# xkuubix/MonteCarlo-Gated-MIL

Measured on AMD Instinct MI355X. Metric: bags/sec × MCDO-samples (T=100) at N=2048,d=512; 1/2/4/8-GPU + %HBM roofline, higher is better.
Workload: dtype bf16

## Files before the change

montecarlo-gated-mil_amd/csrc/mcgmil_kernels.h:

```cpp
#pragma once
#include "mcgmil_device.h"

namespace mcgmil {

struct GateParams {
    const void* H;
    long long ldh;
    const int32_t* bag_off;
    int B, T, L, D, C, G, P;
    long long total_samples;
    const void* Wp;
    uint32_t wp_bytes;
    const float* bv;
    const float* bu;
    const float* wa;
    const float* ba;
    float sf, sa;
    uint32_t thr_f, thr_a;
    uint32_t thrx_f;
    uint32_t k0, k1;
    uint32_t bag_base;
    int t_base;
    const uint32_t* bag_ids;
    const int32_t* tile_bag;
    int uniform_rows;
    const uint8_t* keep_feat;
    const uint8_t* keep_att;
    float* logits;
    float* zz;
    float* Y;
    float* A;
    const int32_t* region_off;
    int region_t;
    unsigned long long* stamps;
    unsigned long long* clock;
    long long tile_row0;
};

constexpr int kClockSlots = 1024;
__device__ __forceinline__ void clock_probe(const GateParams& p, int i) {
    if (p.clock && threadIdx.x == 0 && blockIdx.x < (unsigned)kClockSlots) {
        const unsigned long long t = __builtin_amdgcn_s_memtime();
        const unsigned long long r = __builtin_amdgcn_s_memrealtime();
        p.clock[(size_t)blockIdx.x * 4 + 2 * i] = t;
        p.clock[(size_t)blockIdx.x * 4 + 2 * i + 1] = r;
    }
}

#ifdef MCGMIL_STAMPS
#define MCGMIL_STAMP(p, i)                                                                 \
    do {                                                                                    \
        __builtin_amdgcn_sched_barrier(0);                                                  \
        if (threadIdx.x == 0 && (p).stamps)                                                 \
            (p).stamps[(size_t)blockIdx.x * 8 + (i)] = __builtin_amdgcn_s_memtime();        \
        __builtin_amdgcn_sched_barrier(0);                                                  \
    } while (0)
#else
#define MCGMIL_STAMP(p, i) do {} while (0)
#endif


constexpr int kGateThreads = 512;
constexpr int kGateWaves = kGateThreads / kWave;
constexpr int kRowInfo = 6;


template <int BM, int RV = BM>
__device__ __forceinline__ void fill_row_table(const GateParams& p, long long R0, int* rinfo) {
    const int tid = threadIdx.x;
    if (tid >= BM) return;
    const long long R = tid < RV ? R0 + tid : p.total_samples;
    int hrow = -1, t = 0, n = 0, bag = 0, Nb = 0;
    const bool narrow = p.total_samples <= 0xFFFFFFFFll;
    if (R < p.total_samples && p.uniform_rows > 0) {
        const long long per_bag = (long long)p.T * p.uniform_rows;
        Nb = p.uniform_rows;
        if (narrow) {
            const uint32_t r = (uint32_t)R, pb = (uint32_t)per_bag;
            bag = (int)(r / pb);
            const uint32_t local = r - (uint32_t)bag * pb;
            t = (int)(local / (uint32_t)Nb);
            n = (int)(local - (uint32_t)t * (uint32_t)Nb);
        } else {
            bag = (int)(R / per_bag);
            const long long local = R - (long long)bag * per_bag;
            t = (int)(local / Nb);
            n = (int)(local - (long long)t * Nb);
        }
        hrow = bag * Nb + n;
    } else if (R < p.total_samples) {
        if (p.tile_bag) {
            bag = p.tile_bag[R0 / BM];
            while ((long long)p.T * p.bag_off[bag + 1] <= R) ++bag;
        } else {
            bag = find_bag(p.bag_off, p.B, p.T, R);
        }
        const int ob = p.bag_off[bag];
        Nb = p.bag_off[bag + 1] - ob;
        const long long local = R - (long long)p.T * ob;
        if (narrow) {
            t = (int)((uint32_t)local / (uint32_t)Nb);
            n = (int)((uint32_t)local - (uint32_t)t * (uint32_t)Nb);
        } else {
            t = (int)(local / Nb);
            n = (int)(local - (long long)t * Nb);
        }
        hrow = ob + n;
    }
    int* ri = rinfo + kRowInfo * tid;
    ri[0] = hrow; ri[1] = t; ri[2] = n; ri[3] = bag; ri[4] = Nb;
    ri[5] = (int)(p.bag_ids ? p.bag_ids[bag] : p.bag_base + (uint32_t)bag);
}

#ifndef MCGMIL_KERNELS_TEMPLATES_ONLY
__global__ void plan_tiles_kernel(const int32_t* bag_off, int B, int T, long long total_samples,
                                  int BM, long long tiles, int32_t* tile_bag) {
    const long long i = (long long)blockIdx.x * blockDim.x + threadIdx.x;
    if (i >= tiles) return;
    const long long R = i * BM;
    tile_bag[i] = R < total_samples ? find_bag(bag_off, B, T, R) : 0;
}
#endif

__device__ __forceinline__ float gated_product_scaled(float ax, float by) {
    ax = fminf(fmaxf(ax, -43.280851226668903f), 43.280851226668903f);
    const float a = __builtin_amdgcn_exp2f(ax);
    const float b = __builtin_amdgcn_exp2f(by);
    const float ia = 1.0f + a;
    return (1.0f - a) * __builtin_amdgcn_rcpf(fmaf(ia, b, ia));
}

#ifndef MCGMIL_DIAG
#define MCGMIL_DIAG 0
#endif
#ifndef MCGMIL_PHILOX_ROUNDS
#define MCGMIL_PHILOX_ROUNDS 10
#endif

constexpr float kM2Log2e = -2.8853900817779268f;
constexpr float kMLog2e = -1.4426950408889634f;

struct HeadVec { f32x4 bv, bu, wa; };

template <int PPW>
__device__ __forceinline__ void load_head_vectors(const GateParams& p, int q0, int lane,
                                                  HeadVec (&hv)[PPW]) {
    const int DB = p.D >> 4;
#pragma unroll
    for (int jp = 0; jp < PPW; ++jp) {
        const int q = q0 + jp < p.P ? q0 + jp : p.P - 1;
        const int g = q / DB, db = q - g * DB;
        const int d0 = db * 16 + 4 * (lane >> 4);
        hv[jp].bv = *reinterpret_cast<const f32x4*>(p.bv + (size_t)g * p.D + d0) * kM2Log2e;
        hv[jp].bu = *reinterpret_cast<const f32x4*>(p.bu + (size_t)g * p.D + d0) * kMLog2e;
        hv[jp].wa = *reinterpret_cast<const f32x4*>(p.wa + (size_t)g * p.D + d0);
    }
}

template <int RT, int PPW, int MAXC, bool ONE_CLASS, int RTV = RT>
__device__ __forceinline__ void fold_pairs(const GateParams& p, const f32x4 (&acc)[RT][2 * PPW],
                                           int q0, int lane, float (&part)[MAXC][RT],
                                           const HeadVec* pre = nullptr) {
    const int DB = p.D >> 4;
    const float av_s = p.sf * kM2Log2e, au_s = p.sf * kMLog2e;
#pragma unroll
    for (int jp = 0; jp < PPW; ++jp) {
        const int q = q0 + jp;
        if (q >= p.P) break;
        const int g = q / DB, db = q - g * DB;
        const int d0 = db * 16 + 4 * (lane >> 4);
        f32x4 bvv, buv;
        f32x4 coef[MAXC];
        if (ONE_CLASS && pre) {
            bvv = pre[jp].bv;
            buv = pre[jp].bu;
            coef[0] = pre[jp].wa;
#pragma unroll
            for (int c = 1; c < MAXC; ++c) coef[c] = f32x4{0.f, 0.f, 0.f, 0.f};
        } else {
            bvv = *reinterpret_cast<const f32x4*>(p.bv + (size_t)g * p.D + d0);
            buv = *reinterpret_cast<const f32x4*>(p.bu + (size_t)g * p.D + d0);
            bvv *= kM2Log2e;
            buv *= kMLog2e;
#pragma unroll
            for (int c = 0; c < MAXC; ++c) {
                const int cc = ONE_CLASS ? g : c;
                const bool use = ONE_CLASS ? (c == 0) : ((c < p.C) && (p.G == 1 || c == g));
                const f32x4 w = *reinterpret_cast<const f32x4*>(p.wa + (size_t)(use ? cc : 0) * p.D + d0);
                coef[c] = use ? w : f32x4{0.f, 0.f, 0.f, 0.f};
            }
        }
#pragma unroll
        for (int rt = 0; rt < RTV; ++rt) {
#pragma unroll
            for (int v = 0; v < 4; ++v) {
                const float ax = fmaf(acc[rt][2 * jp][v], av_s, bvv[v]);
                const float by = fmaf(acc[rt][2 * jp + 1][v], au_s, buv[v]);
                if constexpr (ONE_CLASS) {
#if MCGMIL_DIAG & 8
                    part[0][rt] = fmaf(fmaf(ax, coef[0][v], by), ax, part[0][rt]);
                    continue;
#endif
                    const float a = __builtin_amdgcn_exp2f(fminf(fmaxf(ax, -43.280851226668903f),
                                                                 43.280851226668903f));
                    const float b = __builtin_amdgcn_exp2f(by);
                    const float ia = 1.0f + a;
                    const float r = __builtin_amdgcn_rcpf(fmaf(ia, b, ia));
                    part[0][rt] = fmaf(fmaf(-a, coef[0][v], coef[0][v]), r, part[0][rt]);
                } else {
                    const float pr = gated_product_scaled(ax, by);
#pragma unroll
                    for (int c = 0; c < MAXC; ++c) part[c][rt] = fmaf(pr, coef[c][v], part[c][rt]);
                }
            }
        }
    }
}

template <int BM, int MAXC>
__host__ __device__ constexpr int red_floats() { return kGateWaves * MAXC * 4 * BM; }

template <int BM, int MAXC, int ROWS = 16>
__device__ __forceinline__ void finish_scores(const GateParams& p, long long R0,
                                              float (&part)[MAXC][BM / ROWS], f32x4 zacc,
                                              bool zwave, float* red, float* zred,
                                              const int* rinfo, int one_class, int waves_per_gate,
                                              bool have_keep, bool keep, float* lg_out,
                                              float* z_out, long long obase) {
    constexpr int RT = BM / ROWS;
    constexpr int NG = 64 / ROWS;
    const int tid = threadIdx.x, lane = tid & 63, wave = tid >> 6;
    const int ncls = one_class < 0 ? MAXC : 1;
#pragma unroll
    for (int c = 0; c < MAXC; ++c) {
        if (c >= ncls) break;
        const int cls = one_class < 0 ? c : one_class;
        if (cls >= MAXC) break;
        float* dst = red + ((size_t)(wave * MAXC + cls) * NG + lane / ROWS) * BM + (lane % ROWS);
#pragma unroll
        for (int q = 0; q < RT; ++q) dst[ROWS * q] = part[c][q];
    }
    if (zwave && lane < 16) {
#pragma unroll
        for (int c = 0; c < MAXC; ++c) zred[c * BM + wave * 16 + lane] = zacc[c];
    }
    MCGMIL_STAMP(p, 5);
    __syncthreads();
    MCGMIL_STAMP(p, 6);
    const int r = wave * 16 + (lane & 15), c = lane >> 4;
    if (r >= BM || c >= p.C) return;
    const int* ri = rinfo + kRowInfo * r;
    if (ri[0] < 0) return;
    float s = 0.f;
    const int nw = waves_per_gate ? waves_per_gate : kGateWaves;
    for (int k = 0; k < nw; ++k) {
        const int w = waves_per_gate ? c * waves_per_gate + k : k;
        const float* src = red + (size_t)(w * MAXC + c) * NG * BM + r;
#pragma unroll
        for (int g = 0; g < NG; ++g) s += src[g * BM];
    }
    s += p.ba[c];
    const int t = ri[1], n = ri[2], bag = ri[3], Nb = ri[4];
    if (p.keep_att) {
        const size_t abase = (size_t)p.T * p.C * (size_t)p.bag_off[bag];
        keep = p.keep_att[abase + ((size_t)t * p.C + c) * Nb + n] != 0;
    } else if (!have_keep) {
        keep = attention_keep(p.k0, p.k1, (uint32_t)ri[5], (uint32_t)(p.t_base + t), (uint32_t)c,
                              (uint32_t)n, p.thr_a);
    }
    const size_t o = (size_t)(R0 + r - obase) * p.C + c;
    lg_out[o] = s * (keep ? p.sa : 0.f);
    z_out[o] = zred[c * BM + r] * p.sf;
}

constexpr int kSoftmaxRows = 16;

#ifndef MCGMIL_NT_A
#define MCGMIL_NT_A 1
#endif
__device__ __forceinline__ void store_a(float* dst, float v) {
#if MCGMIL_NT_A
    __builtin_nontemporal_store(v, dst);
#else
    *dst = v;
#endif
}

__device__ __forceinline__ void softmax_group(int ltid, bool active, int Nb, int C, const float* lg,
                                              const float* zz, float* Ao, float* Yo, float* sred) {
    const int tid = ltid, lane = ltid & 63, wave = ltid >> 6;
    if (Nb == 0) {
        if (active && tid < C) Yo[tid] = 0.f;
        return;
    }
    const int Nl = active ? Nb : 0;
    if (C == 2 && Nb <= 256 * kSoftmaxRows) {
        float (*sred2)[4] = reinterpret_cast<float (*)[4]>(sred);
        float e0[kSoftmaxRows], e1[kSoftmaxRows];
        float2 zr[kSoftmaxRows];
        float m0 = -INFINITY, m1 = -INFINITY;
#pragma unroll
        for (int k = 0; k < kSoftmaxRows; ++k) {
            const int n = tid + 256 * k;
            float2 l = make_float2(-INFINITY, -INFINITY);
            zr[k] = make_float2(0.f, 0.f);
            if (n < Nl) {
                l = *reinterpret_cast<const float2*>(lg + (size_t)n * 2);
                zr[k] = *reinterpret_cast<const float2*>(zz + (size_t)n * 2);
            }
            e0[k] = l.x;
            e1[k] = l.y;
            m0 = fmaxf(m0, e0[k]);
            m1 = fmaxf(m1, e1[k]);
        }
        m0 = wave_max(m0);
        m1 = wave_max(m1);
        if (lane == 0) { sred2[0][wave] = m0; sred2[1][wave] = m1; }
        __syncthreads();
        m0 = fmaxf(fmaxf(sred2[0][0], sred2[0][1]), fmaxf(sred2[0][2], sred2[0][3]));
        m1 = fmaxf(fmaxf(sred2[1][0], sred2[1][1]), fmaxf(sred2[1][2], sred2[1][3]));
        __syncthreads();
        float s0 = 0.f, y0 = 0.f, s1 = 0.f, y1 = 0.f;
#pragma unroll
        for (int k = 0; k < kSoftmaxRows; ++k) {
            const int n = tid + 256 * k;
            if (n < Nl) {
                const float2 z = zr[k];
                e0[k] = expf(e0[k] - m0);
                e1[k] = expf(e1[k] - m1);
                s0 += e0[k];
                s1 += e1[k];
                y0 = fmaf(e0[k], z.x, y0);
                y1 = fmaf(e1[k], z.y, y1);
            }
        }
        s0 = wave_sum(s0);
        y0 = wave_sum(y0);
        s1 = wave_sum(s1);
        y1 = wave_sum(y1);
        if (lane == 0) {
            sred2[0][wave] = s0; sred2[1][wave] = y0; sred2[2][wave] = s1; sred2[3][wave] = y1;
        }
        __syncthreads();
        s0 = (sred2[0][0] + sred2[0][1]) + (sred2[0][2] + sred2[0][3]);
        y0 = (sred2[1][0] + sred2[1][1]) + (sred2[1][2] + sred2[1][3]);
        s1 = (sred2[2][0] + sred2[2][1]) + (sred2[2][2] + sred2[2][3]);
        y1 = (sred2[3][0] + sred2[3][1]) + (sred2[3][2] + sred2[3][3]);
        __syncthreads();
        const float inv0 = 1.0f / s0, inv1 = 1.0f / s1;
        if (Ao) {
            float* Ao1 = Ao + Nb;
#pragma unroll
            for (int k = 0; k < kSoftmaxRows; ++k) {
                const int n = tid + 256 * k;
                if (n < Nl) {
                    store_a(Ao + n, e0[k] * inv0);
                    store_a(Ao1 + n, e1[k] * inv1);
                }
            }
        }
        if (active && tid == 0) { Yo[0] = y0 * inv0; Yo[1] = y1 * inv1; }
        return;
    }
    float (*sr)[4] = reinterpret_cast<float (*)[4]>(sred);
    for (int c = 0; c < C; ++c) {
        if (Nb <= 256 * kSoftmaxRows) {
            float e[kSoftmaxRows];
            float m = -INFINITY;
#pragma unroll
            for (int k = 0; k < kSoftmaxRows; ++k) {
                const int n = tid + 256 * k;
                e[k] = n < Nl ? lg[(size_t)n * C + c] : -INFINITY;
                m = fmaxf(m, e[k]);
            }
            m = wave_max(m);
            if (lane == 0) sr[0][wave] = m;
            __syncthreads();
            m = fmaxf(fmaxf(sr[0][0], sr[0][1]), fmaxf(sr[0][2], sr[0][3]));
            __syncthreads();
            float s = 0.f, y = 0.f;
#pragma unroll
            for (int k = 0; k < kSoftmaxRows; ++k) {
                const int n = tid + 256 * k;
                if (n < Nl) {
                    e[k] = expf(e[k] - m);
                    s += e[k];
                    y = fmaf(e[k], zz[(size_t)n * C + c], y);
                }
            }
            s = wave_sum(s);
            y = wave_sum(y);
            if (lane == 0) { sr[0][wave] = s; sr[1][wave] = y; }
            __syncthreads();
            s = (sr[0][0] + sr[0][1]) + (sr[0][2] + sr[0][3]);
            y = (sr[1][0] + sr[1][1]) + (sr[1][2] + sr[1][3]);
            __syncthreads();
            const float inv = 1.0f / s;
            if (Ao) {
                float* Aoc = Ao + (size_t)c * Nb;
#pragma unroll
                for (int k = 0; k < kSoftmaxRows; ++k) {
                    const int n = tid + 256 * k;
                    if (n < Nl) store_a(Aoc + n, e[k] * inv);
                }
            }
            if (active && tid == 0) Yo[c] = y * inv;
            continue;
        }
        float m = -INFINITY;
        for (int n = tid; n < Nl; n += 256) m = fmaxf(m, lg[(size_t)n * C + c]);
        m = wave_max(m);
        if (lane == 0) sr[0][wave] = m;
        __syncthreads();
        m = fmaxf(fmaxf(sr[0][0], sr[0][1]), fmaxf(sr[0][2], sr[0][3]));
        __syncthreads();
        float s = 0.f, y = 0.f;
        for (int n = tid; n < Nl; n += 256) {
            const size_t o = (size_t)n * C + c;
            const float e = expf(lg[o] - m);
            s += e;
            y = fmaf(e, zz[o], y);
        }
        s = wave_sum(s);
        y = wave_sum(y);
        if (lane == 0) { sr[0][wave] = s; sr[1][wave] = y; }
        __syncthreads();
        s = (sr[0][0] + sr[0][1]) + (sr[0][2] + sr[0][3]);
        y = (sr[1][0] + sr[1][1]) + (sr[1][2] + sr[1][3]);
        __syncthreads();
        const float inv = 1.0f / s;
        if (Ao) {
            float* Aoc = Ao + (size_t)c * Nb;
            for (int n = tid; n < Nl; n += 256) store_a(Aoc + n, expf(lg[(size_t)n * C + c] - m) * inv);
        }
        if (active && tid == 0) Yo[c] = y * inv;
    }
}

#ifndef MCGMIL_KERNELS_TEMPLATES_ONLY
__global__ __launch_bounds__(256) void softmax_pool_kernel(const int32_t* bag_off, int T, int C,
                                                           const float* logits, const float* zz,
                                                           float* Y, float* A) {
    __shared__ float sred[16];
    const int t = blockIdx.x, b = blockIdx.y;
    const int ob = bag_off[b];
    const int Nb = bag_off[b + 1] - ob;
    const size_t R0 = (size_t)T * ob + (size_t)t * Nb;
    softmax_group(threadIdx.x, true, Nb, C, logits + R0 * C, zz + R0 * C,
                  A ? A + (size_t)T * C * ob + (size_t)t * C * Nb : nullptr,
                  Y + ((size_t)b * T + t) * C, sred);
}
#endif

template <typename E> struct Raw;
template <> struct Raw<__bf16> { uint4 v; };
template <> struct Raw<float> { f32x4 lo, hi; };
__device__ __forceinline__ Raw<__bf16> load_raw(const __bf16* p) {
    Raw<__bf16> r; r.v = *reinterpret_cast<const uint4*>(p); return r;
}
__device__ __forceinline__ Raw<float> load_raw(const float* p) {
    Raw<float> r;
    r.lo = *reinterpret_cast<const f32x4*>(p);
    r.hi = *reinterpret_cast<const f32x4*>(p + 4);
    return r;
}
__device__ __forceinline__ void store_masked(const Raw<__bf16>& h, uint32_t kb, __bf16* dst) {
    uint4 v = h.v;
    v.x &= ((kb & 1u) ? 0x0000FFFFu : 0u) | ((kb & 2u) ? 0xFFFF0000u : 0u);
    v.y &= ((kb & 4u) ? 0x0000FFFFu : 0u) | ((kb & 8u) ? 0xFFFF0000u : 0u);
    v.z &= ((kb & 16u) ? 0x0000FFFFu : 0u) | ((kb & 32u) ? 0xFFFF0000u : 0u);
    v.w &= ((kb & 64u) ? 0x0000FFFFu : 0u) | ((kb & 128u) ? 0xFFFF0000u : 0u);
    *reinterpret_cast<uint4*>(dst) = v;
}
__device__ __forceinline__ void store_masked(const Raw<float>& h, uint32_t kb, float* dst) {
    f32x4 a = h.lo, b = h.hi;
    a.x = (kb & 1u) ? a.x : 0.f;   a.y = (kb & 2u) ? a.y : 0.f;
    a.z = (kb & 4u) ? a.z : 0.f;   a.w = (kb & 8u) ? a.w : 0.f;
    b.x = (kb & 16u) ? b.x : 0.f;  b.y = (kb & 32u) ? b.y : 0.f;
    b.z = (kb & 64u) ? b.z : 0.f;  b.w = (kb & 128u) ? b.w : 0.f;
    *reinterpret_cast<f32x4*>(dst) = a;
    *reinterpret_cast<f32x4*>(dst + 4) = b;
}

__device__ __forceinline__ void store_dropped(const Raw<__bf16>& h, uint4 o, uint32_t thrx,
                                              uint32_t inval, __bf16* dst) {
    uint4 v = h.v;
    v.x = __builtin_amdgcn_bitop3_b32(v.x, drop_mask16x2_flipped(o.x, thrx), inval, 0x10);
    v.y = __builtin_amdgcn_bitop3_b32(v.y, drop_mask16x2(o.y, thrx), inval, 0x10);
    v.z = __builtin_amdgcn_bitop3_b32(v.z, drop_mask16x2_flipped(o.z, thrx), inval, 0x10);
    v.w = __builtin_amdgcn_bitop3_b32(v.w, drop_mask16x2(o.w, thrx), inval, 0x10);
    *reinterpret_cast<uint4*>(dst) = v;
}
__device__ __forceinline__ uint32_t keep_lo(uint32_t m) { return ~(uint32_t)((int32_t)(m << 16) >> 16); }
__device__ __forceinline__ uint32_t keep_hi(uint32_t m) { return ~(uint32_t)((int32_t)m >> 16); }
__device__ __forceinline__ void store_dropped(const Raw<float>& h, uint4 o, uint32_t thrx,
                                              uint32_t inval, float* dst) {
    const uint32_t m0 = drop_mask16x2_flipped(o.x, thrx) | inval, m1 = drop_mask16x2(o.y, thrx) | inval;
    const uint32_t m2 = drop_mask16x2_flipped(o.z, thrx) | inval, m3 = drop_mask16x2(o.w, thrx) | inval;
    f32x4 a = h.lo, b = h.hi;
    a.x = __uint_as_float(__float_as_uint(a.x) & keep_lo(m0));
    a.y = __uint_as_float(__float_as_uint(a.y) & keep_hi(m0));
    a.z = __uint_as_float(__float_as_uint(a.z) & keep_lo(m1));
    a.w = __uint_as_float(__float_as_uint(a.w) & keep_hi(m1));
    b.x = __uint_as_float(__float_as_uint(b.x) & keep_lo(m2));
    b.y = __uint_as_float(__float_as_uint(b.y) & keep_hi(m2));
    b.z = __uint_as_float(__float_as_uint(b.z) & keep_lo(m3));
    b.w = __uint_as_float(__float_as_uint(b.w) & keep_hi(m3));
    *reinterpret_cast<f32x4*>(dst) = a;
    *reinterpret_cast<f32x4*>(dst + 4) = b;
}

constexpr int kPipeBM = 128;
#ifndef MCGMIL_VPM
#define MCGMIL_VPM 2
#endif
constexpr int VPM = MCGMIL_VPM;
#ifndef MCGMIL_SCHED
#define MCGMIL_SCHED 0
#endif
constexpr int HD = 2;
template <typename E>
__host__ __device__ constexpr int pipe_slots() { return 2; }

template <typename E, int MAXC>
__host__ __device__ constexpr size_t pipe_lds_bytes() {
    return (size_t)pipe_slots<E>() * kPipeBM * 32 * sizeof(E) + (size_t)red_floats<kPipeBM, MAXC>() * 4 +
           (size_t)MAXC * kPipeBM * 4 + (size_t)kRowInfo * kPipeBM * 4;
}

template <typename E>
__device__ __forceinline__ void load_classifier_lds(__amdgpu_buffer_rsrc_t wrs, uint32_t zsoff, int KS, E* zw) {
    for (int i = threadIdx.x; i < KS * 64; i += kGateThreads)
        *reinterpret_cast<f32x4*>(zw + (size_t)i * 8) = __builtin_bit_cast(
            f32x4, __builtin_amdgcn_raw_buffer_load_b128(wrs, (uint32_t)i * 8u * (uint32_t)sizeof(E), zsoff, 0));
}

template <typename E, int PPW, int MAXC, bool REPLAY, bool ONE_CLASS, bool EARLY_HV = true,
          bool ZL = false, bool ZLOAD = true, int RTV = kPipeBM / 16>
__device__ __forceinline__ void pipe_tile(const GateParams& p, long long R0, E* Xs, float* red,
                                          float* zred, const int* rinfo, float* lg_out,
                                          float* z_out, long long obase, E* zw = nullptr) {
    constexpr int BM = kPipeBM;
    constexpr int RT = BM / 16;
    constexpr int NJ = 2 * PPW;
    constexpr int SLOT = RT * 64 * 8;
    const int tid = threadIdx.x, lane = tid & 63, wave = tid >> 6;
    const int KS = p.L >> 5;

    const int* ri = rinfo + kRowInfo * (wave * 16 + (lane & 15));
    const int hrow = ri[0];
    const bool valid = hrow >= 0;
    const int kq = lane >> 4;
    const E* hsrc = reinterpret_cast<const E*>(p.H) + (size_t)(valid ? hrow : 0) * p.ldh + kq * 8;
    const uint32_t cn = (uint32_t)ri[2], ct = (uint32_t)(p.t_base + ri[1]), cb = (uint32_t)ri[5];
    const uint8_t* kfe = REPLAY ? p.keep_feat + (size_t)(valid ? R0 + wave * 16 + (lane & 15) : 0) *
                                                    (p.L >> 3) + kq
                                : nullptr;

    const uint32_t inval = valid ? 0u : 0xFFFFFFFFu;
    auto stage = [&](int s, const Raw<E>& h, E* slot) {
        if constexpr (REPLAY) {
            const uint32_t kb = kfe[(size_t)(s < KS ? s : KS - 1) * 4];
            store_masked(h, kb & ~inval, slot + tid * 8);
        } else {
#if MCGMIL_DIAG & 4
            const uint4 o = make_uint4(cn * 0x9E3779B9u + (uint32_t)s, ct ^ cb, cn + ct, (uint32_t)s * 77u);
#else
            const uint4 o = philox4x32_10<true, MCGMIL_PHILOX_ROUNDS>((uint32_t)(s * 4 + kq), cn, ct, cb, p.k0, p.k1);
#endif
            store_dropped(h, o, p.thrx_f, inval, slot + tid * 8);
        }
    };

    const __amdgpu_buffer_rsrc_t wrs = make_rsrc(p.Wp, p.wp_bytes);
    const uint32_t tile_bytes = (uint32_t)KS * 512u * (uint32_t)sizeof(E);
    constexpr uint32_t kStepBytes = 512u * (uint32_t)sizeof(E);
    const int q0 = __builtin_amdgcn_readfirstlane(wave) * PPW;
    uint32_t wsoff[NJ];
#pragma unroll
    for (int j = 0; j < NJ; ++j) {
        int q = q0 + (j >> 1);
        q = q < p.P ? q : p.P - 1;
        wsoff[j] = (uint32_t)(2 * q + (j & 1)) * tile_bytes;
    }
    const uint32_t zsoff = (uint32_t)(2 * p.P) * tile_bytes;
    const uint32_t lane_b = (uint32_t)lane * 8u * (uint32_t)sizeof(E);
    auto wfrag = [&](uint32_t soff) { return load_frag_buf<E>(wrs, lane_b, soff); };

    f32x4 acc[RT][NJ];
#pragma unroll
    for (int rt = 0; rt < RT; ++rt)
#pragma unroll
        for (int j = 0; j < NJ; ++j) acc[rt][j] = f32x4{0.f, 0.f, 0.f, 0.f};
    f32x4 zacc = {0.f, 0.f, 0.f, 0.f};

    auto kstep = [&](int s, const E* cur, E* nxt, const Frag<E> (&w)[NJ], const Frag<E>& z,
                     Frag<E> (&wn)[NJ], Frag<E>& zn, const Raw<E>& h, Raw<E>& hn) {
        const int s1 = s + 1 < KS ? s + 1 : KS - 1;
        const int sh = s + HD < KS ? s + HD : KS - 1;
#if MCGMIL_DIAG & 2
#pragma unroll
        for (int j = 0; j < NJ; ++j) wn[j] = w[j];
        zn = z;
#else
#pragma unroll
        for (int j = 0; j < NJ; ++j) wn[j] = wfrag(wsoff[j] + (uint32_t)s1 * kStepBytes);
        if constexpr (!ZL) zn = wfrag(zsoff + (uint32_t)s1 * kStepBytes);
#endif
#if MCGMIL_DIAG & 1
        hn = h;
#else
        if (RTV == RT || wave < RTV) hn = load_raw(hsrc + (size_t)sh * 32);
#endif
#pragma unroll
        for (int rt = 0; rt < RTV; ++rt) {
            const Frag<E> x = load_frag(cur + (size_t)(rt * 64 + lane) * 8);
#pragma unroll
            for (int j = 0; j < NJ; ++j) acc[rt][j] = mma(w[j], x, acc[rt][j]);
        }
        const Frag<E> xz = load_frag(cur + (size_t)tid * 8);
        if constexpr (ZL) zacc = mma(load_frag(zw + (size_t)(s * 64 + lane) * 8), xz, zacc);
        else zacc = mma(z, xz, zacc);
        if (RTV == RT || wave < RTV) stage(s + 1, h, nxt);
        if constexpr (sizeof(E) == 2 && PPW == 2) {
#if MCGMIL_SCHED == 1
            __builtin_amdgcn_sched_group_barrier(0x020, NJ + 2, 0);
            __builtin_amdgcn_sched_group_barrier(0x100, 3, 0);
#pragma unroll
            for (int rt = 0; rt < RT; ++rt) {
#pragma unroll
                for (int j = 0; j < NJ; ++j) {
                    __builtin_amdgcn_sched_group_barrier(0x008, 1, 0);
                    __builtin_amdgcn_sched_group_barrier(0x002, VPM, 0);
                }
                if (rt + 2 < RT) __builtin_amdgcn_sched_group_barrier(0x100, 1, 0);
            }
            __builtin_amdgcn_sched_group_barrier(0x008, 1, 0);
            __builtin_amdgcn_sched_group_barrier(0x002, VPM, 0);
#else
#pragma unroll
            for (int i = 0; i < RTV * NJ + 1; ++i) {
                __builtin_amdgcn_sched_group_barrier(0x008, 1, 0);
                __builtin_amdgcn_sched_group_barrier(0x002, VPM, 0);
            }
#endif
        }
#if MCGMIL_DIAG & 128
        asm volatile("s_waitcnt lgkmcnt(0)" ::: "memory");
#else
        __syncthreads();
#endif
    };

    constexpr bool kEarlyHV = EARLY_HV && ONE_CLASS && sizeof(E) == 2;
    HeadVec hvec[PPW];
    {
        Frag<E> wA[NJ], wB[NJ], zA, zB;
        Raw<E> hA{}, hB{};
        if (RTV == RT || wave < RTV) {
            hA = load_raw(hsrc);
            hB = load_raw(hsrc + 32);
        }
#pragma unroll
        for (int j = 0; j < NJ; ++j) wA[j] = wfrag(wsoff[j]);
        if constexpr (ZL) {
            if constexpr (ZLOAD) load_classifier_lds<E>(wrs, zsoff, KS, zw);
        } else {
            zA = wfrag(zsoff);
        }
        if (RTV == RT || wave < RTV) stage(0, hA, Xs);
        __syncthreads();
        MCGMIL_STAMP(p, 2);

        if constexpr (kEarlyHV) load_head_vectors<PPW>(p, q0, lane, hvec);
        kstep(0, Xs, Xs + SLOT, wA, zA, wB, zB, hB, hA);
        kstep(1, Xs + SLOT, Xs, wB, zB, wA, zA, hA, hB);
#if MCGMIL_DIAG & 16
        if (KS > 1000)
#endif
        for (int s = 2; s < KS; s += 2) {
            kstep(s, Xs, Xs + SLOT, wA, zA, wB, zB, hB, hA);
            kstep(s + 1, Xs + SLOT, Xs, wB, zB, wA, zA, hA, hB);
        }
    }
    MCGMIL_STAMP(p, 3);

    float part[MAXC][RT];
#pragma unroll
    for (int c = 0; c < MAXC; ++c)
#pragma unroll
        for (int rt = 0; rt < RT; ++rt) part[c][rt] = 0.f;
    fold_pairs<RT, PPW, MAXC, ONE_CLASS, RTV>(p, acc, q0, lane, part, kEarlyHV ? hvec : nullptr);
    MCGMIL_STAMP(p, 4);
    const int one_class = ONE_CLASS ? (q0 < p.P ? q0 / (p.D >> 4) : MAXC) : -1;
    finish_scores<BM, MAXC>(p, R0, part, zacc, true, red, zred, rinfo, one_class,
                            ONE_CLASS ? (p.D >> 4) / PPW : 0, false, true, lg_out, z_out, obase);
    MCGMIL_STAMP(p, 7);
}

#ifndef MCGMIL_XCD_TILES
#define MCGMIL_XCD_TILES 1
#endif
__device__ __forceinline__ long long xcd_tile(unsigned b, unsigned n, int bags) {
#if MCGMIL_XCD_TILES
    const unsigned x = b & 7u, q = n >> 3, r = n & 7u;
    const unsigned l = (x < r ? x * (q + 1) : r * (q + 1) + (x - r) * q) + (b >> 3);
    return (long long)(bags >= 8 ? l : b);
#else
    (void)n;
    (void)bags;
    return (long long)b;
#endif
}

template <typename E, int PPW, int MAXC, bool REPLAY, bool ONE_CLASS, bool PROBE = false, int RTV = kPipeBM / 16>
__global__ __launch_bounds__(kGateThreads) void gate_pipe_kernel(const GateParams p) {
    extern __shared__ __attribute__((aligned(16))) unsigned char smem[];
    constexpr int BM = kPipeBM;
    E* Xs = reinterpret_cast<E*>(smem);
    float* red = reinterpret_cast<float*>(smem + (size_t)pipe_slots<E>() * BM * 32 * sizeof(E));
    float* zred = red + red_floats<BM, MAXC>();
    int* rinfo = reinterpret_cast<int*>(zred + MAXC * BM);
    const long long R0 = RTV == BM / 16 ? xcd_tile(blockIdx.x, gridDim.x, p.B) * BM
                                        : p.tile_row0 + (long long)blockIdx.x * (16 * RTV);

    if constexpr (PROBE) clock_probe(p, 0);
    MCGMIL_STAMP(p, 0);
    fill_row_table<BM, 16 * RTV>(p, R0, rinfo);
    __syncthreads();
    MCGMIL_STAMP(p, 1);
    pipe_tile<E, PPW, MAXC, REPLAY, ONE_CLASS, true, false, true, RTV>(p, R0, Xs, red, zred, rinfo, p.logits,
                                                                       p.zz, 0);
    if constexpr (PROBE) clock_probe(p, 1);
}

#ifndef MCGMIL_FUSED_XCD
#define MCGMIL_FUSED_XCD 1
#endif
#ifndef MCGMIL_FUSED_EARLY_HV
#define MCGMIL_FUSED_EARLY_HV 0
#endif
#ifndef MCGMIL_FUSED_NMAJOR
#define MCGMIL_FUSED_NMAJOR 1
#endif
#ifndef MCGMIL_FUSED_CAP
#define MCGMIL_FUSED_CAP 4096
#endif
template <int MAXC>
__host__ __device__ constexpr int fused_cap() { return MAXC <= 2 ? MCGMIL_FUSED_CAP : MCGMIL_FUSED_CAP / 4; }

template <typename E, int MAXC>
__host__ __device__ constexpr size_t fused_lds_bytes() {
    return pipe_lds_bytes<E, MAXC>() + (size_t)kRowInfo * kPipeBM * 4
           + (size_t)2 * fused_cap<MAXC>() * MAXC * 4
           + (size_t)2 * 16 * 4 + 64;
}

#ifndef MCGMIL_FUSED_ZL
#define MCGMIL_FUSED_ZL 1
#endif
template <typename E>
__host__ __device__ constexpr bool fused_zl() { return MCGMIL_FUSED_ZL && sizeof(E) == 2; }
template <typename E, int MAXC>
__host__ __device__ constexpr size_t fused_kernel_lds_bytes(int L) {
    return fused_lds_bytes<E, MAXC>() + (fused_zl<E>() ? (size_t)(L / 32) * 512 * sizeof(E) : 0);
}

__host__ __device__ inline int region_t_groups(int Nb, int T, int cap) {
    if (Nb <= 0) return T;
    if (Nb > cap) return 1;
    const int ts = cap / Nb;
    return ts < T ? ts : T;
}

struct Region {
    int bag, t0, t1, Nb, ob;
    int ntiles;
    long long S, rows;
};

__device__ __forceinline__ int region_tile(const Region& rg, int i) {
#if MCGMIL_FUSED_NMAJOR
    const int G = rg.t1 - rg.t0;
    if (G > 1 && rg.Nb % kPipeBM == 0) return (i % G) * (rg.Nb / kPipeBM) + i / G;
#endif
    return i;
}

__device__ __forceinline__ GateParams reload_kernarg_params(const GateParams& p) {
#if __HIP_DEVICE_COMPILE__
    typedef __attribute__((address_space(4))) const GateParams* KernargParams;
    KernargParams q = (KernargParams)__builtin_amdgcn_kernarg_segment_ptr();
    asm volatile("" : "+s"(q));
    return *q;
#else
    return p;
#endif
}

__device__ __forceinline__ bool decode_region(const GateParams& p, int g, int cap, Region& rg) {
    int b, j, ts;
    if (p.uniform_rows > 0) {
        ts = p.region_t;
        const int rpb = (p.T + ts - 1) / ts;
        if (MCGMIL_FUSED_XCD && (p.B & 7) == 0) {
            const int k = g >> 3;
            b = 8 * (k / rpb) + (g & 7);
            j = k - (k / rpb) * rpb;
        } else {
            b = g / rpb;
            j = g - b * rpb;
        }
        if (b >= p.B) return false;
    } else {
        if (g >= p.region_off[p.B]) return false;
        b = find_bag(p.region_off, p.B, 1, g);
        j = g - p.region_off[b];
        ts = region_t_groups(p.bag_off[b + 1] - p.bag_off[b], p.T, cap);
    }
    rg.bag = b;
    rg.ob = p.bag_off[b];
    rg.Nb = p.bag_off[b + 1] - rg.ob;
    rg.t0 = j * ts;
    rg.t1 = rg.t0 + ts < p.T ? rg.t0 + ts : p.T;
    rg.S = (long long)p.T * rg.ob + (long long)rg.t0 * rg.Nb;
    rg.rows = (long long)(rg.t1 - rg.t0) * rg.Nb;
    rg.ntiles = (int)((rg.rows + kPipeBM - 1) / kPipeBM);
    return true;
}

template <int BM>
__device__ __forceinline__ void fill_row_table_region(const GateParams& p, const Region& rg,
                                                      long long R0, int* rinfo) {
    const int tid = threadIdx.x;
    if (tid >= BM) return;
    const long long rho = R0 + tid - rg.S;
    int hrow = -1, t = 0, n = 0;
    if (rho < rg.rows) {
        const uint32_t r = (uint32_t)rho;
        const uint32_t tt = r / (uint32_t)rg.Nb;
        n = (int)(r - tt * (uint32_t)rg.Nb);
        t = rg.t0 + (int)tt;
        hrow = rg.ob + n;
    }
    int* ri = rinfo + kRowInfo * tid;
    ri[0] = hrow; ri[1] = t; ri[2] = n; ri[3] = rg.bag; ri[4] = rg.Nb;
    ri[5] = (int)(p.bag_ids ? p.bag_ids[rg.bag] : p.bag_base + (uint32_t)rg.bag);
}


template <typename E, int PPW, int MAXC, bool ONE_CLASS, bool PROBE = false>
__global__ __launch_bounds__(kGateThreads) void gate_fused_kernel(const GateParams p) {
    extern __shared__ __attribute__((aligned(16))) unsigned char smem[];
    constexpr int BM = kPipeBM;
    constexpr int CAP = fused_cap<MAXC>();
    E* Xs = reinterpret_cast<E*>(smem);
    float* red = reinterpret_cast<float*>(smem + (size_t)pipe_slots<E>() * BM * 32 * sizeof(E));
    float* zred = red + red_floats<BM, MAXC>();
    int* rinfo = reinterpret_cast<int*>(zred + MAXC * BM);
    float* slg = reinterpret_cast<float*>(rinfo + 2 * kRowInfo * BM);
    float* szz = slg + CAP * MAXC;
    float* sred = szz + CAP * MAXC;

#if MCGMIL_DIAG & 64
    {
        const long long R0 = (long long)blockIdx.x * BM;
        fill_row_table<BM>(p, R0, rinfo);
        __syncthreads();
        pipe_tile<E, PPW, MAXC, false, ONE_CLASS>(p, R0, Xs, red, zred, rinfo, p.logits, p.zz, 0);
        return;
    }
#endif
    Region rg;
    if (!decode_region(p, (int)blockIdx.x, CAP, rg)) return;
    if constexpr (PROBE) clock_probe(p, 0);
    const int ntiles = (int)((rg.rows + BM - 1) / BM);
    Region* srg = reinterpret_cast<Region*>(sred + 32);
    if (threadIdx.x == 0) *srg = rg;
    __syncthreads();
    E* zw = reinterpret_cast<E*>(smem + fused_lds_bytes<E, MAXC>());
    if constexpr (fused_zl<E>())
        load_classifier_lds<E>(make_rsrc(p.Wp, p.wp_bytes), (uint32_t)(2 * p.P) * (uint32_t)(p.L >> 5) * 512u *
                                   (uint32_t)sizeof(E), p.L >> 5, zw);
    for (int i = 0; i < ntiles; ++i) {
        Region* qr = srg;
        asm volatile("" : "+v"(qr));
        const GateParams pt = reload_kernarg_params(p);
        int* ri = rinfo + (i & 1) * kRowInfo * BM;
        MCGMIL_STAMP(pt, 0);
        {
            const Region r = *qr;
            fill_row_table_region<BM>(pt, r, r.S + (long long)region_tile(r, i) * BM, ri);
        }
        __syncthreads();
        MCGMIL_STAMP(pt, 1);
        const Region r = *qr;
        const bool lds = r.Nb <= CAP;
        pipe_tile<E, PPW, MAXC, false, ONE_CLASS, MCGMIL_FUSED_EARLY_HV, fused_zl<E>(), false>(
            pt, r.S + (long long)region_tile(r, i) * BM, Xs, red, zred, ri, lds ? slg : pt.logits,
            lds ? szz : pt.zz, lds ? r.S : 0, zw);
    }
    __syncthreads();
#if MCGMIL_DIAG & 32
    if (ntiles >= 0) return;
#endif
    rg = *srg;
    const bool in_lds = rg.Nb <= CAP;

    const int G = rg.t1 - rg.t0;
    const int half = threadIdx.x >> 8, ltid = threadIdx.x & 255;
    for (int j0 = 0; j0 < G; j0 += 2) {
        const bool act = j0 + half < G;
        const int j = act ? j0 + half : j0;
        const long long row0 = (long long)j * rg.Nb;
        const float* lgj = in_lds ? slg + row0 * p.C : p.logits + (rg.S + row0) * p.C;
        const float* zzj = in_lds ? szz + row0 * p.C : p.zz + (rg.S + row0) * p.C;
        float* Ao = p.A ? p.A + (size_t)p.T * p.C * rg.ob + (size_t)(rg.t0 + j) * p.C * rg.Nb : nullptr;
        float* Yo = p.Y + ((size_t)rg.bag * p.T + rg.t0 + j) * p.C;
        softmax_group(ltid, act, rg.Nb, p.C, lgj, zzj, Ao, Yo, sred + half * 16);
    }
    if constexpr (PROBE) clock_probe(p, 1);
}

template <int BM>
__host__ __device__ constexpr int gate_row_info_ints() { return kRowInfo * BM; }

template <typename E, int BM, int MAXC>
__host__ __device__ constexpr size_t gate_lds_bytes(int L) {
    const size_t tile = (size_t)BM * L * sizeof(E), red = (size_t)red_floats<BM, MAXC>() * 4;
    return (tile > red ? tile : red) + (size_t)MAXC * BM * 4 + (size_t)gate_row_info_ints<BM>() * 4;
}

template <typename E, int BM, int PPW, int MAXC>
__global__ __launch_bounds__(kGateThreads) void gate_scores_kernel(const GateParams p) {
    extern __shared__ __attribute__((aligned(16))) unsigned char smem[];
    constexpr int RT = BM / 16;
    constexpr int NJ = 2 * PPW;
    const int tid = threadIdx.x;
    const int lane = tid & 63;
    const int wave = tid >> 6;
    const int L = p.L;
    const int KS = L >> 5;
    const int LC = L >> 3;

    E* Xs = reinterpret_cast<E*>(smem);
    float* red = reinterpret_cast<float*>(smem);
    const size_t tile_bytes = (size_t)BM * L * sizeof(E), red_bytes = (size_t)red_floats<BM, MAXC>() * 4;
    float* zred = reinterpret_cast<float*>(smem + (tile_bytes > red_bytes ? tile_bytes : red_bytes));
    int* rinfo = reinterpret_cast<int*>(zred + MAXC * BM);
    const long long R0 = (long long)blockIdx.x * BM;

    fill_row_table<BM>(p, R0, rinfo);
    __syncthreads();

    {
        const E* H = reinterpret_cast<const E*>(p.H);
        const int items = BM * LC;
        for (int i = tid; i < items; i += kGateThreads) {
            const int blk = i >> 6, slot = i & 63;
            const int rt = blk / KS, ks = blk - rt * KS;
            const int r = rt * 16 + (slot & 15);
            const int kc = ks * 4 + (slot >> 4);
            E* dst = Xs + ((size_t)blk * 64 + slot) * 8;
            const int* ri = rinfo + kRowInfo * r;
            const int hrow = ri[0];
            if (hrow < 0) {
                store_zero8(dst);
                continue;
            }
            uint32_t kb;
            if (p.keep_feat) {
                kb = p.keep_feat[(size_t)(R0 + r) * LC + kc];
            } else {
                const uint4 o = philox4x32_10((uint32_t)kc, (uint32_t)ri[2],
                                              (uint32_t)(p.t_base + ri[1]), (uint32_t)ri[5],
                                              p.k0, p.k1);
                kb = keep_byte(o, p.thr_f);
            }
            load_masked(H + (size_t)hrow * p.ldh + (size_t)kc * 8, kb, dst);
        }
    }
    __syncthreads();

    const E* Wp = reinterpret_cast<const E*>(p.Wp);
    const int pairs_per_pass = kGateWaves * PPW;
    const int npass = (p.P + pairs_per_pass - 1) / pairs_per_pass;
    const size_t tile_elems = (size_t)KS * 512;

    float part[MAXC][RT];
#pragma unroll
    for (int c = 0; c < MAXC; ++c)
#pragma unroll
        for (int rt = 0; rt < RT; ++rt) part[c][rt] = 0.f;
    f32x4 zacc = {0.f, 0.f, 0.f, 0.f};
    const bool zwave = wave < RT;

    for (int pass = 0; pass < npass; ++pass) {
        const int q0 = pass * pairs_per_pass + wave * PPW;
        const bool active = q0 < p.P;
        const bool doz = (pass == 0) && zwave;
        if (!active && !doz) continue;

        f32x4 acc[RT][NJ];
#pragma unroll
        for (int rt = 0; rt < RT; ++rt)
#pragma unroll
            for (int j = 0; j < NJ; ++j) acc[rt][j] = f32x4{0.f, 0.f, 0.f, 0.f};

        const E* wbase[NJ];
#pragma unroll
        for (int j = 0; j < NJ; ++j) {
            int q = q0 + (j >> 1);
            q = q < p.P ? q : p.P - 1;
            wbase[j] = Wp + (size_t)(2 * q + (j & 1)) * tile_elems + lane * 8;
        }
        const E* zbase = Wp + (size_t)(2 * p.P) * tile_elems + lane * 8;

        Frag<E> wcur[NJ], wnxt[NJ];
        Frag<E> zcur = zero_frag<E>(), znxt = zero_frag<E>();
#pragma unroll
        for (int j = 0; j < NJ; ++j) wcur[j] = active ? load_frag(wbase[j]) : zero_frag<E>();
        if (doz) zcur = load_frag(zbase);

        for (int ks = 0; ks < KS; ++ks) {
            if (ks + 1 < KS) {
#pragma unroll
                for (int j = 0; j < NJ; ++j)
                    if (active) wnxt[j] = load_frag(wbase[j] + (size_t)(ks + 1) * 512);
                if (doz) znxt = load_frag(zbase + (size_t)(ks + 1) * 512);
            }
#pragma unroll
            for (int rt = 0; rt < RT; ++rt) {
                const Frag<E> x = load_frag(Xs + ((size_t)(rt * KS + ks) * 64 + lane) * 8);
                if (active) {
#pragma unroll
                    for (int j = 0; j < NJ; ++j) acc[rt][j] = mma(wcur[j], x, acc[rt][j]);
                }
                if (doz && rt == wave) zacc = mma(zcur, x, zacc);
            }
#pragma unroll
            for (int j = 0; j < NJ; ++j) wcur[j] = wnxt[j];
            zcur = znxt;
        }
        if (!active) continue;
        fold_pairs<RT, PPW, MAXC, false>(p, acc, q0, lane, part);
    }
    __syncthreads();
    finish_scores<BM, MAXC>(p, R0, part, zacc, zwave, red, zred, rinfo, -1, 0, false, true,
                            p.logits, p.zz, 0);
}

constexpr int kStatOuts = 64, kStatGroups = 8, kStatThreads = kStatOuts * kStatGroups;
#ifndef MCGMIL_KERNELS_TEMPLATES_ONLY
__global__ __launch_bounds__(kStatThreads) void bag_stats_kernel(const int32_t* bag_off, int B, int T, int C,
                                                                 long long total_rows, int stat_blocks,
                                                                 const float* A, const float* Y,
                                                                 float* A_mean, float* A_var, float* P_mean) {
    if ((int)blockIdx.x < stat_blocks) {
        __shared__ double ssum[kStatGroups][kStatOuts], ssq[kStatGroups][kStatOuts];
        const int o = threadIdx.x % kStatOuts, grp = threadIdx.x / kStatOuts;
        const long long i = (long long)blockIdx.x * kStatOuts + o;
        const bool live = i < total_rows * C;
        double s = 0.0, ss = 0.0;
        if (live) {
            const int bag = find_bag(bag_off, B, C, i);
            const int ob = bag_off[bag];
            const int Nb = bag_off[bag + 1] - ob;
            const long long local = i - (long long)C * ob;
            const int c = (int)(local / Nb);
            const int n = (int)(local - (long long)c * Nb);
            const float* a = A + (size_t)T * C * ob + (size_t)c * Nb + n;
            const size_t step = (size_t)C * Nb;
#pragma unroll 4
            for (int t = grp; t < T; t += kStatGroups) {
                const double v = a[(size_t)t * step];
                s += v;
                ss += v * v;
            }
        }
        ssum[grp][o] = s;
        ssq[grp][o] = ss;
        __syncthreads();
        if (grp != 0 || !live) return;
        s = ssum[0][o];
        ss = ssq[0][o];
#pragma unroll
        for (int g = 1; g < kStatGroups; ++g) {
            s += ssum[g][o];
            ss += ssq[g][o];
        }
        const double mean = s / T;
        if (A_mean) A_mean[i] = (float)mean;
        if (A_var) A_var[i] = T > 1 ? (float)fmax((ss - s * mean) / (T - 1), 0.0) : NAN;
        return;
    }
    if (!P_mean) return;
    const int b = ((int)blockIdx.x - stat_blocks) * (kStatThreads / kWave) + (int)(threadIdx.x / kWave);
    const int lane = threadIdx.x % kWave;
    if (b >= B) return;
    double acc[4] = {0.0, 0.0, 0.0, 0.0};
    for (int t = lane; t < T; t += kWave) {
        const float* y = Y + ((size_t)b * T + t) * C;
        float v[4];
#pragma unroll
        for (int k = 0; k < 4; ++k) v[k] = k < C ? y[k] : -INFINITY;
        const float m = fmaxf(fmaxf(v[0], v[1]), fmaxf(v[2], v[3]));
        float e[4], sum = 0.f;
#pragma unroll
        for (int k = 0; k < 4; ++k) {
            e[k] = k < C ? expf(v[k] - m) : 0.f;
            sum += e[k];
        }
#pragma unroll
        for (int k = 0; k < 4; ++k) acc[k] += (double)(e[k] / sum);
    }
#pragma unroll
    for (int k = 0; k < 4; ++k) acc[k] = wave_sum_d(acc[k]);
    if (lane < C) {
        const double a = lane == 0 ? acc[0] : lane == 1 ? acc[1] : lane == 2 ? acc[2] : acc[3];
        P_mean[(size_t)b * C + lane] = (float)(a / T);
    }
}
#endif

template <typename E>
__global__ void pack_weights_kernel(const float* Wv, const float* Wu, const float* wk, int L, int D,
                                    int C, int P, E* out) {
    const int KS = L >> 5;
    const size_t total = (size_t)(2 * P + 1) * KS * 512;
    const int DB = D >> 4;
    for (size_t i = (size_t)blockIdx.x * blockDim.x + threadIdx.x; i < total;
         i += (size_t)gridDim.x * blockDim.x) {
        const int j = (int)(i & 7);
        const int lane = (int)((i >> 3) & 63);
        const size_t blk = i >> 9;
        const int ks = (int)(blk % KS);
        const int tile = (int)(blk / KS);
        const int col = lane & 15;
        const int k = ks * 32 + 8 * (lane >> 4) + j;
        float v;
        if (tile < 2 * P) {
            const int q = tile >> 1;
            const int g = q / DB, db = q - g * DB;
            const float* W = (tile & 1) ? Wu : Wv;
            v = W[((size_t)g * D + db * 16 + col) * L + k];
        } else {
            v = col < C ? wk[(size_t)col * L + k] : 0.f;
        }
        out[i] = static_cast<E>(v);
    }
}

#ifndef MCGMIL_KERNELS_TEMPLATES_ONLY
__global__ void feature_keep_kernel(const int32_t* bag_off, int B, int T, int LC,
                                    long long total_samples, uint32_t k0, uint32_t k1,
                                    uint32_t bag_base, const uint32_t* bag_ids, int t_base,
                                    uint32_t thr, uint8_t* out) {
    const long long total = total_samples * LC;
    for (long long i = (long long)blockIdx.x * blockDim.x + threadIdx.x; i < total;
         i += (long long)gridDim.x * blockDim.x) {
        const long long R = i / LC;
        const int kc = (int)(i - R * LC);
        const int bag = find_bag(bag_off, B, T, R);
        const int ob = bag_off[bag];
        const int Nb = bag_off[bag + 1] - ob;
        const long long local = R - (long long)T * ob;
        const int t = (int)(local / Nb);
        const int n = (int)(local - (long long)t * Nb);
        const uint32_t bagc = bag_ids ? bag_ids[bag] : bag_base + (uint32_t)bag;
        const uint4 o = philox4x32_10((uint32_t)kc, (uint32_t)n, (uint32_t)(t_base + t), bagc,
                                      k0, k1);
        out[i] = (uint8_t)keep_byte(o, thr);
    }
}
#endif

#ifndef MCGMIL_KERNELS_TEMPLATES_ONLY
__global__ void attention_keep_kernel(const int32_t* bag_off, int B, int T, int C,
                                      long long total, uint32_t k0, uint32_t k1,
                                      uint32_t bag_base, const uint32_t* bag_ids, int t_base,
                                      uint32_t thr, uint8_t* out) {
    for (long long i = (long long)blockIdx.x * blockDim.x + threadIdx.x; i < total;
         i += (long long)gridDim.x * blockDim.x) {
        const int bag = find_bag(bag_off, B, (long long)T * C, i);
        const int ob = bag_off[bag];
        const int Nb = bag_off[bag + 1] - ob;
        const long long local = i - (long long)T * C * ob;
        const int t = (int)(local / ((long long)C * Nb));
        const long long rem = local - (long long)t * C * Nb;
        const int c = (int)(rem / Nb);
        const int n = (int)(rem - (long long)c * Nb);
        const uint32_t bagc = bag_ids ? bag_ids[bag] : bag_base + (uint32_t)bag;
        out[i] = attention_keep(k0, k1, bagc, (uint32_t)(t_base + t), (uint32_t)c, (uint32_t)n,
                                thr) ? 1 : 0;
    }
}
#endif

}
```

Baseline: 914,500.

## Peel last K-steps of gate pipeline and defer head-vector loads into tail

Peels the final two k-steps of the software-pipelined MFMA loop so the clamped over-fetch of weights and H rows past the end is dropped. In the last step, the freed load slots are used to fetch the head bias and attention vectors (optionally also the attention-keep mask), and explicit scheduling barriers interleave these with the remaining MFMAs. Index clamping is removed on the peeled path. The aim is to cut wasted tail memory traffic and move the epilogue vector loads off the critical path. The cost is more template specialization and code size, and the change only applies to certain E/PPW/ONE_CLASS combinations.

```diff
diff --git a/montecarlo-gated-mil_amd/csrc/mcgmil_kernels.h b/montecarlo-gated-mil_amd/csrc/mcgmil_kernels.h
--- a/montecarlo-gated-mil_amd/csrc/mcgmil_kernels.h
+++ b/montecarlo-gated-mil_amd/csrc/mcgmil_kernels.h
@@ -142,7 +142,7 @@
 
 struct HeadVec { f32x4 bv, bu, wa; };
 
-template <int PPW>
+template <int PPW, bool SCALE = true>
 __device__ __forceinline__ void load_head_vectors(const GateParams& p, int q0, int lane,
                                                   HeadVec (&hv)[PPW]) {
     const int DB = p.D >> 4;
@@ -151,9 +151,21 @@
         const int q = q0 + jp < p.P ? q0 + jp : p.P - 1;
         const int g = q / DB, db = q - g * DB;
         const int d0 = db * 16 + 4 * (lane >> 4);
-        hv[jp].bv = *reinterpret_cast<const f32x4*>(p.bv + (size_t)g * p.D + d0) * kM2Log2e;
-        hv[jp].bu = *reinterpret_cast<const f32x4*>(p.bu + (size_t)g * p.D + d0) * kMLog2e;
+        hv[jp].bv = *reinterpret_cast<const f32x4*>(p.bv + (size_t)g * p.D + d0);
+        hv[jp].bu = *reinterpret_cast<const f32x4*>(p.bu + (size_t)g * p.D + d0);
         hv[jp].wa = *reinterpret_cast<const f32x4*>(p.wa + (size_t)g * p.D + d0);
+        if constexpr (SCALE) {
+            hv[jp].bv *= kM2Log2e;
+            hv[jp].bu *= kMLog2e;
+        }
+    }
+}
+template <int PPW>
+__device__ __forceinline__ void scale_head_vectors(HeadVec (&hv)[PPW]) {
+#pragma unroll
+    for (int jp = 0; jp < PPW; ++jp) {
+        hv[jp].bv *= kM2Log2e;
+        hv[jp].bu *= kMLog2e;
     }
 }
 
@@ -535,14 +547,37 @@
             f32x4, __builtin_amdgcn_raw_buffer_load_b128(wrs, (uint32_t)i * 8u * (uint32_t)sizeof(E), zsoff, 0));
 }
 
-template <typename E, int PPW, int MAXC, bool REPLAY, bool ONE_CLASS, bool EARLY_HV = true,
-          bool ZL = false, bool ZLOAD = true, int RTV = kPipeBM / 16>
+#ifndef MCGMIL_TAIL_PEEL
+#define MCGMIL_TAIL_PEEL 1
+#endif
+#ifndef MCGMIL_TAIL_KEEP
+#define MCGMIL_TAIL_KEEP 0
+#endif
+#ifndef MCGMIL_TAIL_FUSED
+#define MCGMIL_TAIL_FUSED 0
+#endif
+constexpr int kTailFull = 0, kTailNoH = 1, kTailLast = 2;
+template <int M> struct TailMode { static constexpr int value = M; };
+constexpr int kHvFold = 0;
+constexpr int kHvEarly = 1;
+constexpr int kHvTail = 2;
+#ifndef MCGMIL_PIPE_HV
+#define MCGMIL_PIPE_HV 2
+#endif
+#ifndef MCGMIL_FUSED_HV
+#define MCGMIL_FUSED_HV 2
+#endif
+
+template <typename E, int PPW, int MAXC, bool REPLAY, bool ONE_CLASS, int HV_MODE = kHvEarly,
+          bool ZL = false, bool ZLOAD = true, int RTV = kPipeBM / 16, bool TILE_LOOP = false>
 __device__ __forceinline__ void pipe_tile(const GateParams& p, long long R0, E* Xs, float* red,
                                           float* zred, const int* rinfo, float* lg_out,
                                           float* z_out, long long obase, E* zw = nullptr) {
     constexpr int BM = kPipeBM;
     constexpr int RT = BM / 16;
     constexpr int NJ = 2 * PPW;
+    constexpr bool kPeel = MCGMIL_TAIL_PEEL && (!TILE_LOOP || MCGMIL_TAIL_FUSED) &&
+                           !(sizeof(E) == 2 && PPW == 2 && !ONE_CLASS) && !(sizeof(E) == 4 && PPW == 2);
     constexpr int SLOT = RT * 64 * 8;
     const int tid = threadIdx.x, lane = tid & 63, wave = tid >> 6;
     const int KS = p.L >> 5;
@@ -560,7 +595,7 @@
     const uint32_t inval = valid ? 0u : 0xFFFFFFFFu;
     auto stage = [&](int s, const Raw<E>& h, E* slot) {
         if constexpr (REPLAY) {
-            const uint32_t kb = kfe[(size_t)(s < KS ? s : KS - 1) * 4];
+            const uint32_t kb = kfe[(size_t)(kPeel || s < KS ? s : KS - 1) * 4];
             store_masked(h, kb & ~inval, slot + tid * 8);
         } else {
 #if MCGMIL_DIAG & 4
@@ -594,24 +629,37 @@
         for (int j = 0; j < NJ; ++j) acc[rt][j] = f32x4{0.f, 0.f, 0.f, 0.f};
     f32x4 zacc = {0.f, 0.f, 0.f, 0.f};
 
+    constexpr int kHvMode = ONE_CLASS && sizeof(E) == 2 ? (HV_MODE == kHvTail && !kPeel ? kHvFold : HV_MODE)
+                                                        : kHvFold;
+    constexpr bool kTailKeep = kPeel && MCGMIL_TAIL_KEEP && !REPLAY;
+    HeadVec hvec[PPW];
+    bool akeep = false;
     auto kstep = [&](int s, const E* cur, E* nxt, const Frag<E> (&w)[NJ], const Frag<E>& z,
-                     Frag<E> (&wn)[NJ], Frag<E>& zn, const Raw<E>& h, Raw<E>& hn) {
-        const int s1 = s + 1 < KS ? s + 1 : KS - 1;
-        const int sh = s + HD < KS ? s + HD : KS - 1;
+                     Frag<E> (&wn)[NJ], Frag<E>& zn, const Raw<E>& h, Raw<E>& hn, auto tail) {
+        constexpr int TAIL = decltype(tail)::value;
+        const int s1 = kPeel || s + 1 < KS ? s + 1 : KS - 1;
+        const int sh = kPeel || s + HD < KS ? s + HD : KS - 1;
+        if constexpr (TAIL == kTailLast) {
+            if constexpr (kHvMode == kHvTail) load_head_vectors<PPW, false>(p, q0, lane, hvec);
+            if constexpr (kTailKeep) akeep = attention_keep(p.k0, p.k1, cb, ct, (uint32_t)kq, cn, p.thr_a);
+        } else {
 #if MCGMIL_DIAG & 2
 #pragma unroll
-        for (int j = 0; j < NJ; ++j) wn[j] = w[j];
-        zn = z;
+            for (int j = 0; j < NJ; ++j) wn[j] = w[j];
+            zn = z;
 #else
 #pragma unroll
-        for (int j = 0; j < NJ; ++j) wn[j] = wfrag(wsoff[j] + (uint32_t)s1 * kStepBytes);
-        if constexpr (!ZL) zn = wfrag(zsoff + (uint32_t)s1 * kStepBytes);
-#endif
+            for (int j = 0; j < NJ; ++j) wn[j] = wfrag(wsoff[j] + (uint32_t)s1 * kStepBytes);
+            if constexpr (!ZL) zn = wfrag(zsoff + (uint32_t)s1 * kStepBytes);
+#endif
+        }
+        if constexpr (TAIL == kTailFull) {
 #if MCGMIL_DIAG & 1
-        hn = h;
+            hn = h;
 #else
-        if (RTV == RT || wave < RTV) hn = load_raw(hsrc + (size_t)sh * 32);
-#endif
+            if (RTV == RT || wave < RTV) hn = load_raw(hsrc + (size_t)sh * 32);
+#endif
+        }
 #pragma unroll
         for (int rt = 0; rt < RTV; ++rt) {
             const Frag<E> x = load_frag(cur + (size_t)(rt * 64 + lane) * 8);
@@ -621,8 +669,17 @@
         const Frag<E> xz = load_frag(cur + (size_t)tid * 8);
         if constexpr (ZL) zacc = mma(load_frag(zw + (size_t)(s * 64 + lane) * 8), xz, zacc);
         else zacc = mma(z, xz, zacc);
-        if (RTV == RT || wave < RTV) stage(s + 1, h, nxt);
-        if constexpr (sizeof(E) == 2 && PPW == 2) {
+        if constexpr (TAIL != kTailLast) {
+            if (RTV == RT || wave < RTV) stage(s + 1, h, nxt);
+        }
+        if constexpr (sizeof(E) == 2 && PPW == 2 && TAIL == kTailLast) {
+            if constexpr (kHvMode == kHvTail) __builtin_amdgcn_sched_group_barrier(0x020, 3 * PPW, 0);
+#pragma unroll
+            for (int i = 0; i < RTV * NJ + 1; ++i) {
+                __builtin_amdgcn_sched_group_barrier(0x008, 1, 0);
+                __builtin_amdgcn_sched_group_barrier(0x002, VPM, 0);
+            }
+        } else if constexpr (sizeof(E) == 2 && PPW == 2) {
 #if MCGMIL_SCHED == 1
             __builtin_amdgcn_sched_group_barrier(0x020, NJ + 2, 0);
             __builtin_amdgcn_sched_group_barrier(0x100, 3, 0);
@@ -652,8 +709,6 @@
 #endif
     };
 
-    constexpr bool kEarlyHV = EARLY_HV && ONE_CLASS && sizeof(E) == 2;
-    HeadVec hvec[PPW];
     {
         Frag<E> wA[NJ], wB[NJ], zA, zB;
         Raw<E> hA{}, hB{};
@@ -672,16 +727,36 @@
         __syncthreads();
         MCGMIL_STAMP(p, 2);
 
-        if constexpr (kEarlyHV) load_head_vectors<PPW>(p, q0, lane, hvec);
-        kstep(0, Xs, Xs + SLOT, wA, zA, wB, zB, hB, hA);
-        kstep(1, Xs + SLOT, Xs, wB, zB, wA, zA, hA, hB);
+        if constexpr (kHvMode == kHvEarly) load_head_vectors<PPW>(p, q0, lane, hvec);
+        constexpr TailMode<kTailFull> full{};
+        constexpr TailMode<kTailNoH> no_h{};
+        constexpr TailMode<kTailLast> last{};
+        if constexpr (!kPeel) {
+            kstep(0, Xs, Xs + SLOT, wA, zA, wB, zB, hB, hA, full);
+            kstep(1, Xs + SLOT, Xs, wB, zB, wA, zA, hA, hB, full);
 #if MCGMIL_DIAG & 16
-        if (KS > 1000)
-#endif
-        for (int s = 2; s < KS; s += 2) {
-            kstep(s, Xs, Xs + SLOT, wA, zA, wB, zB, hB, hA);
-            kstep(s + 1, Xs + SLOT, Xs, wB, zB, wA, zA, hA, hB);
-        }
+            if (KS > 1000)
+#endif
+            for (int s = 2; s < KS; s += 2) {
+                kstep(s, Xs, Xs + SLOT, wA, zA, wB, zB, hB, hA, full);
+                kstep(s + 1, Xs + SLOT, Xs, wB, zB, wA, zA, hA, hB, full);
+            }
+        } else {
+            if (KS > 2) {
+                kstep(0, Xs, Xs + SLOT, wA, zA, wB, zB, hB, hA, full);
+                kstep(1, Xs + SLOT, Xs, wB, zB, wA, zA, hA, hB, full);
+#if MCGMIL_DIAG & 16
+                if (KS > 1000)
+#endif
+                for (int s = 2; s < KS - 2; s += 2) {
+                    kstep(s, Xs, Xs + SLOT, wA, zA, wB, zB, hB, hA, full);
+                    kstep(s + 1, Xs + SLOT, Xs, wB, zB, wA, zA, hA, hB, full);
+                }
+            }
+            kstep(KS - 2, Xs, Xs + SLOT, wA, zA, wB, zB, hB, hA, no_h);
+            kstep(KS - 1, Xs + SLOT, Xs, wB, zB, wA, zA, hA, hB, last);
+        }
+        if constexpr (kHvMode == kHvTail) scale_head_vectors<PPW>(hvec);
     }
     MCGMIL_STAMP(p, 3);
 
@@ -690,11 +765,12 @@
     for (int c = 0; c < MAXC; ++c)
 #pragma unroll
         for (int rt = 0; rt < RT; ++rt) part[c][rt] = 0.f;
-    fold_pairs<RT, PPW, MAXC, ONE_CLASS, RTV>(p, acc, q0, lane, part, kEarlyHV ? hvec : nullptr);
+    fold_pairs<RT, PPW, MAXC, ONE_CLASS, RTV>(p, acc, q0, lane, part, kHvMode != kHvFold ? hvec : nullptr);
     MCGMIL_STAMP(p, 4);
     const int one_class = ONE_CLASS ? (q0 < p.P ? q0 / (p.D >> 4) : MAXC) : -1;
     finish_scores<BM, MAXC>(p, R0, part, zacc, true, red, zred, rinfo, one_class,
-                            ONE_CLASS ? (p.D >> 4) / PPW : 0, false, true, lg_out, z_out, obase);
+                            ONE_CLASS ? (p.D >> 4) / PPW : 0, kTailKeep, kTailKeep ? akeep : true, lg_out,
+                            z_out, obase);
     MCGMIL_STAMP(p, 7);
 }
 
@@ -729,8 +805,8 @@
     fill_row_table<BM, 16 * RTV>(p, R0, rinfo);
     __syncthreads();
     MCGMIL_STAMP(p, 1);
-    pipe_tile<E, PPW, MAXC, REPLAY, ONE_CLASS, true, false, true, RTV>(p, R0, Xs, red, zred, rinfo, p.logits,
-                                                                       p.zz, 0);
+    pipe_tile<E, PPW, MAXC, REPLAY, ONE_CLASS, MCGMIL_PIPE_HV, false, true, RTV>(p, R0, Xs, red, zred, rinfo,
+                                                                                 p.logits, p.zz, 0);
     if constexpr (PROBE) clock_probe(p, 1);
 }
 
@@ -896,7 +972,7 @@
         MCGMIL_STAMP(pt, 1);
         const Region r = *qr;
         const bool lds = r.Nb <= CAP;
-        pipe_tile<E, PPW, MAXC, false, ONE_CLASS, MCGMIL_FUSED_EARLY_HV, fused_zl<E>(), false>(
+        pipe_tile<E, PPW, MAXC, false, ONE_CLASS, MCGMIL_FUSED_EARLY_HV ? kHvEarly : MCGMIL_FUSED_HV, fused_zl<E>(), false, kPipeBM / 16, true>(
             pt, r.S + (long long)region_tile(r, i) * BM, Xs, red, zred, ri, lds ? slg : pt.logits,
             lds ? szz : pt.zz, lds ? r.S : 0, zw);
     }
```

After: 913,000. No clear change (-0.2%).
